# c0gent/hbbft

Hardware: AMD Instinct MI355X
Metric: verified BLS sig shares/sec (whole node) + combine latency, N=64 f=21 (higher is better)
Workload: dtype u32 limbs (Fp, 14x28-bit); 1 GPU; ThresholdSign share verification, BASELINE configs[1]; batch_per_gpu=65536, streams=2, documents_per_gpu=1024, n_nodes=64, f=21, pairing_impl=auto, parallelism=shard-by-batch x1

## Files before the change

### hbbft_amd/csrc/k_pair.hip

```cpp
#define HS_MULFN static __device__ __noinline__
#include "launch.hpp"
#include "pair_side.hpp"

namespace hbs {

template <bool PLUS1>
HP_D H12 h_exp_abs_x(const H12& base) {
  const uint64_t e = PLUS1 ? hb::X_ABS + 1 : hb::X_ABS;
  H12 r = base;
#pragma unroll 1
  for (int k = 62; k >= 0; k--) {
    r = h12_cyclo_sqr(r);
    if ((e >> k) & 1) r = h12_mul(r, base);
  }
  return r;
}
HP_D H12 h_exp_x(const H12& f) { return h12_conj(h_exp_abs_x<false>(f)); }
HP_D H12 h_exp_xm1(const H12& f) { return h12_conj(h_exp_abs_x<true>(f)); }

HP_D H12 h_final_exp(const H12& f, uint32_t* __restrict__ stash) {
  const H12 f1 = h12_mul(h12_conj(f), h12_inv(f));
  const H12 g = h12_mul(h12_frob2(f1), f1);
  stash12(stash, g);
  H12 a = h_exp_xm1(h_exp_xm1(g));
  const H12 b = h12_mul(h_exp_x(a), h12_frob1(a));
  {
    const H12 gs = unstash12(stash);
    const H12 w = h12_mul(h12_mul(h12_frob2(b), h12_conj(b)), h12_mul(h12_cyclo_sqr(gs), gs));
    stash12(stash, w);
  }
  const H12 c = h_exp_x(h_exp_x(b));
  return h12_mul(c, unstash12(stash));
}

template <bool W1, bool W2, int GEN>
__global__ void __launch_bounds__(256, 2) k_pair_verify(PairArgs a) {
  extern __shared__ uint32_t stash_lds[];
  const int i = (int)((blockIdx.x * 256u + threadIdx.x) >> 1);
  if (i >= a.n) return;
  constexpr bool G1 = GEN == 1, G2 = GEN == 2;
  const bool neg2 = (a.flags & 1) != 0;
  SideStateH A, B;
  const bool ok1 = side_init<W1, G1>(a.s1, i, false, A);
  const bool ok2 = side_init<W2, G2>(a.s2, i, neg2, B);
  if (!ok1 || !ok2) {
    if (lp_even() && a.verdict) a.verdict[i] = 0;
    return;
  }
  H12 f = h12_one();
  int step = 0;
#pragma unroll 1
  for (int b = 62; b >= 0; b--) {
    if (b != 62) f = h12_sqr(f);
    {
      const HLine la = side_line<W1, G1, true>(a.s1, A, step, false);
      const HLine lb = side_line<W2, G2, true>(a.s2, B, step, neg2);
      f = h12_mul_lines(f, la.c0, la.c1, la.c4, lb.c0, lb.c1, lb.c4);
    }
    step++;
    if ((hb::X_ABS >> b) & 1) {
      const HLine la = side_line<W1, G1, false>(a.s1, A, step, false);
      const HLine lb = side_line<W2, G2, false>(a.s2, B, step, neg2);
      f = h12_mul_lines(f, la.c0, la.c1, la.c4, lb.c0, lb.c1, lb.c4);
      step++;
    }
  }
  if (a.flags & 2) f = h12_conj(f);
  const H12 e = h_final_exp(f, stash_lds + threadIdx.x);
  if (a.value_out) {
    uint32_t* o = a.value_out + (size_t)i * 144 + (lp_even() ? 0 : 12);
    fp_to_words(e.c0.c0, o + 0);
    fp_to_words(e.c0.c1, o + 24);
    fp_to_words(e.c0.c2, o + 48);
    fp_to_words(e.c1.c0, o + 72);
    fp_to_words(e.c1.c1, o + 96);
    fp_to_words(e.c1.c2, o + 120);
  }
  const bool one = h12_is_one(e);
  if (lp_even() && a.verdict) a.verdict[i] = one ? 1 : 0;
}

}

namespace hbl {

size_t pair_table_bytes(size_t nq) { return nq * (size_t)hbs::PAIR_STEPS * 2 * hbs::PL_Q4 * 16; }

hipError_t pair_verify(hipStream_t s, int n, const PairSideDesc& d1, const PairSideDesc& d2, int flags,
                       uint8_t* verdict, uint32_t* value_out) {
  if (n <= 0) return hipSuccess;
  hbs::PairArgs a;
  a.n = n;
  const PairSideDesc* d[2] = {&d1, &d2};
  hbs::PairSide* o[2] = {&a.s1, &a.s2};
  for (int k = 0; k < 2; k++) {
    o[k]->p = (const uint32_t*)d[k]->p;
    o[k]->q = (const uint32_t*)d[k]->q;
    o[k]->lines = (const int4*)d[k]->lines;
    o[k]->qinf = d[k]->qinf;
    o[k]->idx = d[k]->idx;
    o[k]->nq = (uint32_t)d[k]->nq;
  }
  a.flags = flags;
  a.verdict = verdict;
  a.value_out = value_out;
  const dim3 grid((unsigned)((2 * (size_t)n + 255) / 256)), block(256);
  const size_t lds = (size_t)hbs::STASH_WORDS * 256 * 4;
  const bool w1 = d1.lines == nullptr, w2 = d2.lines == nullptr;
  const int gen = (d1.p == nullptr) == (d2.p == nullptr) ? 0 : (d1.p == nullptr ? 1 : 2);
#define HBS_PAIR_LAUNCH(G)                                                                 \
  do {                                                                                     \
    if (w1 && w2)                                                                          \
      hipLaunchKernelGGL((hbs::k_pair_verify<true, true, G>), grid, block, lds, s, a);     \
    else if (w1)                                                                           \
      hipLaunchKernelGGL((hbs::k_pair_verify<true, false, G>), grid, block, lds, s, a);    \
    else if (w2)                                                                           \
      hipLaunchKernelGGL((hbs::k_pair_verify<false, true, G>), grid, block, lds, s, a);    \
    else                                                                                   \
      hipLaunchKernelGGL((hbs::k_pair_verify<false, false, G>), grid, block, lds, s, a);   \
  } while (0)
  if (gen == 1)
    HBS_PAIR_LAUNCH(1);
  else if (gen == 2)
    HBS_PAIR_LAUNCH(2);
  else
    HBS_PAIR_LAUNCH(0);
#undef HBS_PAIR_LAUNCH
  return hipGetLastError();
}

}
```

### hbbft_amd/csrc/pfp.hpp

```cpp
#pragma once
#include "sfp.hpp"
#include "words.hpp"

#define HP_D __device__ __forceinline__

namespace hbs {

constexpr int DPP_SWAP = 0xB1;
constexpr int DPP_EVEN = 0xA0;
constexpr int DPP_ODD = 0xF5;

HP_D bool lp_even() { return (threadIdx.x & 1) == 0; }
template <int CTRL>
HP_D int32_t dpp(int32_t v) {
  return __builtin_amdgcn_mov_dpp(v, CTRL, 0xF, 0xF, true);
}
template <int CTRL>
HP_D Fp dpp_fp(const Fp& a) {
  Fp r;
#pragma unroll
  for (int i = 0; i < NL; i++) r.l[i] = dpp<CTRL>(a.l[i]);
  return r;
}

HS_MULFN Fp h_mul_l(HS_P14(x), HS_P14(y)) {
  const Fp a = {{HS_L14(x)}};
  const Fp b = {{HS_L14(y)}};
  const int32_t sm = lp_even() ? -1 : 0;
  int32_t Y[NL], W[NL], Z[NL];
#pragma unroll
  for (int i = 0; i < NL; i++) {
    Y[i] = dpp<DPP_EVEN>(b.l[i]);
    W[i] = dpp<DPP_ODD>(b.l[i]);
    Z[i] = (dpp<DPP_SWAP>(a.l[i]) ^ sm) - sm;
  }
  int32_t m[NL];
  int64_t acc = 0;
  Fp r;
#pragma unroll
  for (int k = 0; k < NL; k++) {
#pragma unroll
    for (int i = 0; i <= k; i++) {
      acc += (int64_t)a.l[i] * Y[k - i];
      acc += (int64_t)Z[i] * W[k - i];
    }
#pragma unroll
    for (int i = 0; i < k; i++) acc += (int64_t)m[i] * (int32_t)P_L[k - i];
    m[k] = mont_digit(acc);
    acc += (int64_t)m[k] * (int32_t)P_L[0];
    acc >>= 28;
  }
#pragma unroll
  for (int k = NL; k < 2 * NL - 1; k++) {
#pragma unroll
    for (int i = k - NL + 1; i < NL; i++) {
      acc += (int64_t)a.l[i] * Y[k - i];
      acc += (int64_t)Z[i] * W[k - i];
      acc += (int64_t)m[i] * (int32_t)P_L[k - i];
    }
    r.l[k - NL] = (int32_t)acc & MASK28;
    acc >>= 28;
  }
  r.l[NL - 1] = (int32_t)acc;
  return r;
}

HP_D Fp h_mul(const Fp& a, const Fp& b) { return h_mul_l(HS_E14(a), HS_E14(b)); }

HP_D Fp h_sqr(const Fp& a) {
  const bool ev = lp_even();
  const Fp pa = dpp_fp<DPP_SWAP>(a);
  Fp x, y;
#pragma unroll
  for (int i = 0; i < NL; i++) {
    x.l[i] = pa.l[i] + (ev ? a.l[i] : pa.l[i]);
    y.l[i] = a.l[i] - (ev ? pa.l[i] : 0);
  }
  return fp_mul(x, y);
}

HP_D Fp h_mul_xi(const Fp& a) {
  const int32_t sm = lp_even() ? -1 : 0;
  const Fp pa = dpp_fp<DPP_SWAP>(a);
  Fp r;
#pragma unroll
  for (int i = 0; i < NL; i++) r.l[i] = a.l[i] + ((pa.l[i] ^ sm) - sm);
  fp_norm(r);
  return r;
}
HP_D Fp h_conj(const Fp& a) {
  const Fp n = fp_neg(a);
  return lp_even() ? a : n;
}
HP_D Fp h_zero() { return fp_zero(); }
HP_D Fp h_one() { return lp_even() ? fp_one() : fp_zero(); }
HP_D Fp h_const(const uint32_t (&c0)[NL], const uint32_t (&c1)[NL]) {
  Fp r;
  const bool ev = lp_even();
#pragma unroll
  for (int i = 0; i < NL; i++) r.l[i] = (int32_t)(ev ? c0[i] : c1[i]);
  return r;
}
HP_D bool lp_both(bool v) { return (v ? 1 : 0) & dpp<DPP_SWAP>(v ? 1 : 0); }
HP_D bool h_is_zero(const Fp& a) { return lp_both(fp_is_zero(a)); }
template <int MODE = 0>
HP_D Fp h_inv_vartime(const Fp& a) {
  const Fp s = fp_sqr(a);
  const Fp n = fp_add(s, dpp_fp<DPP_SWAP>(s));
  uint32_t w[12], p[12], r[12];
  fp_to_words(n, w);
  uint32_t nz = 0;
#pragma unroll
  for (int i = 0; i < 12; i++) nz |= w[i];
  if (nz == 0) return fp_zero();
#pragma unroll
  for (int i = 0; i < 12; i++) p[i] = hb::PM2_W[i];
  p[0] += 2;
  hb::words_inv_vartime<12, MODE>(w, p, r);
  return h_conj(fp_mul(a, fp_from_words(r)));
}

template <int M, int K>
HP_D Fp fp_red_mk(const Fp& t, const Fp& a) {
  const int64_t top = (int64_t)t.l[NL - 1] * M + (int64_t)K * a.l[NL - 1];
  const int32_t q = (int32_t)((top * QINV) >> 32);
  Fp r;
  int64_t acc = 0;
#pragma unroll
  for (int i = 0; i < NL - 1; i++) {
    acc += (int64_t)t.l[i] * M + (int64_t)K * a.l[i] - (int64_t)q * (int32_t)P_L[i];
    r.l[i] = (int32_t)acc & MASK28;
    acc >>= 28;
  }
  r.l[NL - 1] = (int32_t)(acc + top - (int64_t)q * (int32_t)P_L[NL - 1]);
  return r;
}
HP_D Fp fp_red_l(const Fp& t) { return fp_red_mk<1, 0>(t, t); }
HP_D Fp h_add_xi_l(const Fp& s, const Fp& t) {
  const int32_t sm = lp_even() ? -1 : 0;
  const Fp pt = dpp_fp<DPP_SWAP>(t);
  Fp r;
#pragma unroll
  for (int i = 0; i < NL; i++) r.l[i] = s.l[i] + t.l[i] + ((pt.l[i] ^ sm) - sm);
  return r;
}
HP_D Fp fp_sub2l(const Fp& a, const Fp& b, const Fp& c) {
  Fp r;
#pragma unroll
  for (int i = 0; i < NL; i++) r.l[i] = a.l[i] - b.l[i] - c.l[i];
  return r;
}

HP_D Fp h_xi_l(const Fp& t) {
  const int32_t sm = lp_even() ? -1 : 0;
  const Fp pt = dpp_fp<DPP_SWAP>(t);
  Fp r;
#pragma unroll
  for (int i = 0; i < NL; i++) r.l[i] = t.l[i] + ((pt.l[i] ^ sm) - sm);
  return r;
}

struct H6 { Fp c0, c1, c2; };
struct H12 { H6 c0, c1; };

HP_D H6 h6_zero() { return {h_zero(), h_zero(), h_zero()}; }
HP_D H6 h6_one() { return {h_one(), h_zero(), h_zero()}; }
HP_D H6 h6_add(const H6& a, const H6& b) { return {fp_add(a.c0, b.c0), fp_add(a.c1, b.c1), fp_add(a.c2, b.c2)}; }
HP_D H6 h6_sub(const H6& a, const H6& b) { return {fp_sub(a.c0, b.c0), fp_sub(a.c1, b.c1), fp_sub(a.c2, b.c2)}; }
HP_D H6 h6_neg(const H6& a) { return {fp_neg(a.c0), fp_neg(a.c1), fp_neg(a.c2)}; }
HP_D H6 h6_red(const H6& a) { return {fp_reduce(a.c0), fp_reduce(a.c1), fp_reduce(a.c2)}; }
HP_D H6 h6_mul_v(const H6& a) { return {h_mul_xi(a.c2), a.c0, a.c1}; }

HP_D H6 h6_mul(const H6& a, const H6& b) {
  const Fp v1 = h_mul(a.c1, b.c1);
  const Fp v2 = h_mul(a.c2, b.c2);
  const Fp d0 = fp_sub2l(h_mul(fp_addl(a.c1, a.c2), fp_add(b.c1, b.c2)), v1, v2);
  const Fp v0 = h_mul(a.c0, b.c0);
  const Fp c0 = fp_red_l(h_add_xi_l(v0, d0));
  const Fp c1 = fp_red_l(h_add_xi_l(fp_sub2l(h_mul(fp_addl(a.c0, a.c1), fp_add(b.c0, b.c1)), v0, v1), v2));
  const Fp c2 = fp_red_l(fp_addl(fp_sub2l(h_mul(fp_addl(a.c0, a.c2), fp_add(b.c0, b.c2)), v0, v2), v1));
  return {c0, c1, c2};
}
HP_D H6 h6_mul_01(const H6& x, const Fp& a, const Fp& b) {
  const Fp t0 = h_mul(x.c0, a);
  const Fp t1 = h_mul(x.c1, b);
  const Fp u = h_mul(x.c2, b);
  const Fp w = h_mul(x.c2, a);
  const Fp s = h_mul(fp_addl(x.c0, x.c1), fp_add(a, b));
  return {fp_add(t0, h_mul_xi(u)), fp_sub(fp_subl(s, t0), t1), fp_add(t1, w)};
}
HP_D H6 h6_mul_1(const H6& x, const Fp& b) {
  const Fp r0 = h_mul(x.c2, b);
  const Fp r1 = h_mul(x.c0, b);
  const Fp r2 = h_mul(x.c1, b);
  return {h_mul_xi(r0), r1, r2};
}
HP_D H6 h6_inv(const H6& a) {
  const Fp c0 = fp_reduce(fp_sub(h_sqr(a.c0), h_mul_xi(h_mul(a.c1, a.c2))));
  const Fp c1 = fp_reduce(fp_sub(h_mul_xi(h_sqr(a.c2)), h_mul(a.c0, a.c1)));
  const Fp c2 = fp_reduce(fp_sub(h_sqr(a.c1), h_mul(a.c0, a.c2)));
  const Fp t = fp_reduce(fp_add(h_mul(a.c0, c0), h_mul_xi(fp_add(h_mul(a.c2, c1), h_mul(a.c1, c2)))));
  const Fp ti = fp_reduce(h_inv_vartime(t));
  return {h_mul(c0, ti), h_mul(c1, ti), h_mul(c2, ti)};
}

HP_D H12 h12_one() { return {h6_one(), h6_zero()}; }
HP_D H12 h12_conj(const H12& a) { return {a.c0, h6_neg(a.c1)}; }
HP_D H12 h12_red(const H12& a) { return {h6_red(a.c0), h6_red(a.c1)}; }
HP_D H12 h12_kcomb(const H6& t0, const H6& t1, const H6& s) {
  return {{fp_red_l(h_add_xi_l(t0.c0, t1.c2)), fp_red_l(fp_addl(t0.c1, t1.c0)), fp_red_l(fp_addl(t0.c2, t1.c1))},
          {fp_red_l(fp_sub2l(s.c0, t0.c0, t1.c0)), fp_red_l(fp_sub2l(s.c1, t0.c1, t1.c1)),
           fp_red_l(fp_sub2l(s.c2, t0.c2, t1.c2))}};
}

HP_D H12 h12_mul(const H12& a, const H12& b) {
  const H6 t0 = h6_mul(a.c0, b.c0);
  const H6 t1 = h6_mul(a.c1, b.c1);
  const H6 s = h6_mul(h6_add(a.c0, a.c1), h6_add(b.c0, b.c1));
  return h12_kcomb(t0, t1, s);
}
HP_D H12 h12_sqr(const H12& a) {
  const H6 t = h6_mul(a.c0, a.c1);
  const H6 s = h6_mul(h6_add(a.c0, a.c1), h6_red(h6_add(a.c0, h6_mul_v(a.c1))));
  return {{fp_red_l(h_add_xi_l(fp_subl(s.c0, t.c0), fp_subl(fp_zero(), t.c2))), fp_red_l(fp_sub2l(s.c1, t.c1, t.c0)),
           fp_red_l(fp_sub2l(s.c2, t.c2, t.c1))},
          {fp_red_l(fp_addl(t.c0, t.c0)), fp_red_l(fp_addl(t.c1, t.c1)), fp_red_l(fp_addl(t.c2, t.c2))}};
}
HP_D H12 h12_mul_014(const H12& f, const Fp& c0, const Fp& c1, const Fp& c4) {
  const H6 fs = h6_add(f.c0, f.c1);
  const Fp c14 = fp_add(c1, c4);
  const H6 t0 = h6_red(h6_mul_01(f.c0, c0, c1));
  const H6 t1 = h6_red(h6_mul_1(f.c1, c4));
  const H6 s = h6_red(h6_mul_01(fs, c0, c14));
  return h12_red({h6_add(t0, h6_mul_v(t1)), h6_sub(h6_sub(s, t0), t1)});
}
HP_D H6 h6_mul_12(const H6& x, const Fp& b1, const Fp& b2) {
  const Fp u = h_mul(x.c1, b1);
  const Fp w = h_mul(x.c2, b2);
  const Fp c0 = fp_red_l(h_xi_l(fp_sub2l(h_mul(fp_addl(x.c1, x.c2), fp_add(b1, b2)), u, w)));
  const Fp c1 = fp_red_l(h_add_xi_l(h_mul(x.c0, b1), w));
  const Fp c2 = fp_red_l(fp_addl(h_mul(x.c0, b2), u));
  return {c0, c1, c2};
}
HP_D H12 h12_mul_lines(const H12& f, const Fp& a0, const Fp& a1, const Fp& a4, const Fp& b0, const Fp& b1,
                       const Fp& b4) {
  const Fp a0b0 = h_mul(a0, b0);
  const Fp a1b1 = h_mul(a1, b1);
  const Fp a4b4 = h_mul(a4, b4);
  const Fp c11 = fp_red_l(fp_sub2l(h_mul(fp_addl(a0, a4), fp_add(b0, b4)), a0b0, a4b4));
  const Fp c12 = fp_red_l(fp_sub2l(h_mul(fp_addl(a1, a4), fp_add(b1, b4)), a1b1, a4b4));
  const H6 C0 = {fp_red_l(h_add_xi_l(a0b0, a4b4)),
                 fp_red_l(fp_sub2l(h_mul(fp_addl(a0, a1), fp_add(b0, b1)), a0b0, a1b1)), a1b1};
  const H6 t0 = h6_mul(f.c0, C0);
  const H6 t1 = h6_mul_12(f.c1, c11, c12);
  const H6 s = h6_mul(h6_add(f.c0, f.c1), {C0.c0, fp_add(C0.c1, c11), fp_add(C0.c2, c12)});
  return h12_kcomb(t0, t1, s);
}
HP_D H12 h12_inv(const H12& a) {
  const H6 t = h6_red(h6_sub(h6_red(h6_mul(a.c0, a.c0)), h6_red(h6_mul_v(h6_red(h6_mul(a.c1, a.c1))))));
  const H6 ti = h6_red(h6_inv(t));
  return h12_red({h6_mul(a.c0, ti), h6_neg(h6_mul(a.c1, ti))});
}

#define HP_FROB1(K) h_const(hb::FROB1_##K##_C0, hb::FROB1_##K##_C1)
HP_D H12 h12_frob1(const H12& f) {
  H12 r;
  r.c0.c0 = h_conj(f.c0.c0);
  r.c1.c0 = h_mul(h_conj(f.c1.c0), HP_FROB1(1));
  r.c0.c1 = h_mul(h_conj(f.c0.c1), HP_FROB1(2));
  r.c1.c1 = h_mul(h_conj(f.c1.c1), HP_FROB1(3));
  r.c0.c2 = h_mul(h_conj(f.c0.c2), HP_FROB1(4));
  r.c1.c2 = h_mul(h_conj(f.c1.c2), HP_FROB1(5));
  return h12_red(r);
}
HP_D H12 h12_frob2(const H12& f) {
  H12 r;
  r.c0.c0 = f.c0.c0;
  r.c1.c0 = fp_mul(f.c1.c0, fp_const(hb::FROB2_1_C0));
  r.c0.c1 = fp_mul(f.c0.c1, fp_const(hb::FROB2_2_C0));
  r.c1.c1 = fp_mul(f.c1.c1, fp_const(hb::FROB2_3_C0));
  r.c0.c2 = fp_mul(f.c0.c2, fp_const(hb::FROB2_4_C0));
  r.c1.c2 = fp_mul(f.c1.c2, fp_const(hb::FROB2_5_C0));
  return r;
}

HP_D H12 h12_cyclo_sqr(const H12& f) {
  const Fp& a0 = f.c0.c0; const Fp& a2 = f.c0.c1; const Fp& a4 = f.c0.c2;
  const Fp& a1 = f.c1.c0; const Fp& a3 = f.c1.c1; const Fp& a5 = f.c1.c2;
  H12 r;
  {
    const Fp s0 = h_sqr(a0), s3 = h_sqr(a3), s03 = h_sqr(fp_add(a0, a3));
    r.c0.c0 = fp_red_mk<3, -2>(h_add_xi_l(s0, s3), a0);
    r.c1.c1 = fp_red_mk<3, 2>(fp_sub2l(s03, s0, s3), a3);
  }
  {
    const Fp s1 = h_sqr(a1), s4 = h_sqr(a4), s14 = h_sqr(fp_add(a1, a4));
    r.c0.c1 = fp_red_mk<3, -2>(h_add_xi_l(s1, s4), a2);
    r.c1.c2 = fp_red_mk<3, 2>(fp_sub2l(s14, s1, s4), a5);
  }
  {
    const Fp s2 = h_sqr(a2), s5 = h_sqr(a5), s25 = h_sqr(fp_add(a2, a5));
    r.c0.c2 = fp_red_mk<3, -2>(h_add_xi_l(s2, s5), a4);
    r.c1.c0 = fp_red_mk<3, 2>(h_add_xi_l(fp_zero(), fp_sub2l(s25, s2, s5)), a1);
  }
  return r;
}

HP_D bool h12_is_one(const H12& f) {
  bool ok = fp_is_zero(fp_sub(f.c0.c0, h_one()));
  ok = ok && fp_is_zero(f.c0.c1) && fp_is_zero(f.c0.c2);
  ok = ok && fp_is_zero(f.c1.c0) && fp_is_zero(f.c1.c1) && fp_is_zero(f.c1.c2);
  return lp_both(ok);
}

struct HJac { Fp x, y, z; };
struct HLine { Fp c0, c1, c4; };

HP_D HLine h_dbl_step(HJac& T) {
  const Fp A = h_sqr(T.x);
  const Fp B = h_sqr(T.y);
  const Fp C = h_sqr(B);
  const Fp D = fp_lin(2, fp_sub(fp_sub(h_sqr(fp_add(T.x, B)), A), C), 0, C);
  const Fp E = fp_lin(3, A, 0, A);
  const Fp ZZ = h_sqr(T.z);
  HLine l;
  l.c0 = fp_sub(h_mul(E, T.x), fp_add(B, B));
  l.c1 = fp_neg(h_mul(E, ZZ));
  const Fp Z3 = fp_sub(fp_sub(h_sqr(fp_add(T.y, T.z)), B), ZZ);
  l.c4 = h_mul(Z3, ZZ);
  const Fp F = h_sqr(E);
  const Fp X3 = fp_sub(F, fp_add(D, D));
  T.y = fp_sub(h_mul(E, fp_sub(D, X3)), fp_lin(8, C, 0, C));
  T.x = X3;
  T.z = Z3;
  l.c0 = fp_reduce(l.c0);
  T.x = fp_reduce(T.x);
  T.y = fp_reduce(T.y);
  T.z = fp_reduce(T.z);
  return l;
}

HP_D HLine h_add_step(HJac& T, const Fp& xQ, const Fp& yQ) {
  const Fp Z1Z1 = h_sqr(T.z);
  const Fp U2 = h_mul(xQ, Z1Z1);
  const Fp S2 = h_mul(h_mul(yQ, T.z), Z1Z1);
  const Fp H = fp_sub(U2, T.x);
  const Fp r = fp_sub(S2, T.y);
  const Fp HH = h_sqr(H);
  const Fp HHH = h_mul(H, HH);
  const Fp V = h_mul(T.x, HH);
  const Fp X3 = fp_sub(fp_sub(h_sqr(r), HHH), fp_add(V, V));
  const Fp Y3 = fp_sub(h_mul(r, fp_sub(V, X3)), h_mul(T.y, HHH));
  const Fp Z3 = h_mul(T.z, H);
  HLine l;
  l.c0 = fp_reduce(fp_sub(h_mul(r, xQ), h_mul(yQ, Z3)));
  l.c1 = fp_neg(r);
  l.c4 = Z3;
  T.x = fp_reduce(X3);
  T.y = fp_reduce(Y3);
  T.z = Z3;
  return l;
}

struct HProj { Fp x, y, z; };

HP_D HLine h_dbl_step_h(HProj& T) {
  const Fp C = h_sqr(T.z);
  const Fp YZ = h_sqr(fp_add(T.y, T.z));
  const Fp B = h_sqr(T.y);
  const Fp H = fp_sub(fp_sub(YZ, B), C);
  const Fp E = fp_red_mk<12, 0>(h_xi_l(C), C);
  const Fp A = h_mul(T.x, T.y);
  const Fp S = h_sqr(T.x);
  HLine l;
  l.c0 = fp_red_mk<1, -1>(B, E);
  l.c1 = fp_lin(-3, S, 0, S);
  l.c4 = H;
  const Fp Bm = fp_lin(1, B, -3, E);
  const Fp Bp = fp_lin(1, B, 3, E);
  T.x = h_mul(fp_addl(A, A), Bm);
  const Fp EE = h_sqr(E);
  T.y = fp_red_mk<1, -12>(h_sqr(Bp), EE);
  const Fp BH = h_mul(fp_addl(B, B), H);
  T.z = fp_red_mk<2, 0>(BH, BH);
  return l;
}

HP_D HLine h_add_step_h(HProj& T, const Fp& xQ, const Fp& yQ) {
  const Fp th = fp_sub(T.y, h_mul(yQ, T.z));
  const Fp la = fp_sub(T.x, h_mul(xQ, T.z));
  HLine l;
  l.c0 = fp_reduce(fp_sub(h_mul(th, xQ), h_mul(la, yQ)));
  l.c1 = fp_neg(th);
  l.c4 = la;
  const Fp C = h_sqr(th);
  const Fp D = h_sqr(la);
  const Fp E = h_mul(la, D);
  const Fp F = h_mul(T.z, C);
  const Fp G = h_mul(T.x, D);
  const Fp H = fp_lin(1, fp_addl(E, F), -2, G);
  const Fp X3 = h_mul(la, H);
  T.y = fp_reduce(fp_sub(h_mul(th, fp_sub(G, H)), h_mul(E, T.y)));
  T.z = h_mul(T.z, E);
  T.x = X3;
  return l;
}

HP_D void h_g2_load(const uint32_t* __restrict__ w, Fp& x, Fp& y) {
  const int o = lp_even() ? 0 : 12;
  x = fp_from_words(w + o);
  y = fp_from_words(w + 24 + o);
}
HP_D bool words_zero(const uint32_t* __restrict__ w, int n) {
  uint32_t o = 0;
  for (int k = 0; k < n; k++) o |= w[k];
  return o == 0;
}

}
```

Before: 3.360 million shares/s.

## Use compressed cyclotomic squaring with batched decompression in final-exp x-powers

Replaces the plain square-and-multiply exponentiation by |x| in the final exponentiation with Karabina-style compressed cyclotomic squaring. Intermediate powers at set bits are parked, then decompressed using a single batched (Montgomery-trick) inversion before being multiplied together. If a denominator is zero, it falls back to the generic routine. This cuts per-squaring field multiplications, at the cost of one inversion per exponentiation, extra parked state that may raise register or scratch pressure, and a noinline call structure.

```diff
diff --git a/hbbft_amd/csrc/k_pair.hip b/hbbft_amd/csrc/k_pair.hip
--- a/hbbft_amd/csrc/k_pair.hip
+++ b/hbbft_amd/csrc/k_pair.hip
@@ -4,32 +4,119 @@
 
 namespace hbs {
 
-template <bool PLUS1>
-HP_D H12 h_exp_abs_x(const H12& base) {
-  const uint64_t e = PLUS1 ? hb::X_ABS + 1 : hb::X_ABS;
-  H12 r = base;
+constexpr int EXP_TOP = 57;
+constexpr uint64_t EXP_HIGH = hb::X_ABS >> EXP_TOP;
+constexpr int EXP_HIGH_BITS = 64 - EXP_TOP;
+constexpr int EXP_NPARK = __builtin_popcountll(hb::X_ABS) - __builtin_popcountll(EXP_HIGH) + 1;
+static_assert((hb::X_ABS & 1) == 0 && (hb::X_ABS >> 63) == 1 && (EXP_HIGH & 1) == 1 && EXP_NPARK >= 1,
+              "the base is no factor of f^|x|, and the power at bit EXP_TOP is the last one parked");
+struct ExpPark {
+  int32_t c[EXP_NPARK][4][NL];
+  int32_t base[6][NL];
+  int32_t pre[EXP_NPARK][NL];
+};
+
+HP_D void park_fp(int32_t (&d)[NL], const Fp& a) {
+#pragma unroll
+  for (int i = 0; i < NL; i++) d[i] = a.l[i];
+}
+HP_D Fp unpark_fp(const int32_t (&s)[NL]) {
+  Fp r;
+#pragma unroll
+  for (int i = 0; i < NL; i++) r.l[i] = s[i];
+  return r;
+}
+HP_D H12 unpark12(const int32_t (&s)[6][NL]) {
+  return {{unpark_fp(s[0]), unpark_fp(s[1]), unpark_fp(s[2])}, {unpark_fp(s[3]), unpark_fp(s[4]), unpark_fp(s[5])}};
+}
+
+static __device__ __noinline__ void h_exp_gs(const ExpPark& pk, bool plus1, H12& out) {
+  const uint64_t e = hb::X_ABS + (plus1 ? 1 : 0);
+  H12 r = unpark12(pk.base);
 #pragma unroll 1
   for (int k = 62; k >= 0; k--) {
     r = h12_cyclo_sqr(r);
-    if ((e >> k) & 1) r = h12_mul(r, base);
+    if ((e >> k) & 1) r = h12_mul(r, unpark12(pk.base));
+  }
+  out = r;
+}
+
+HP_D H12 h_exp_high(const H12& t) {
+  H12 r = t;
+#pragma unroll 1
+  for (int k = EXP_HIGH_BITS - 2; k >= 0; k--) {
+    r = h12_cyclo_sqr(r);
+    if ((EXP_HIGH >> k) & 1) r = h12_mul(r, t);
   }
   return r;
 }
-HP_D H12 h_exp_x(const H12& f) { return h12_conj(h_exp_abs_x<false>(f)); }
-HP_D H12 h_exp_xm1(const H12& f) { return h12_conj(h_exp_abs_x<true>(f)); }
+
+static __device__ __noinline__ bool h_exp_tail(ExpPark& pk, bool plus1, H12& out) {
+  Fp P;
+#pragma unroll 1
+  for (int j = 0; j < EXP_NPARK; j++) {
+    const Fp d = hc_denom(unpark_fp(pk.c[j][0]));
+    if (j == 0) P = d; else P = h_mul(P, d);
+    park_fp(pk.pre[j], P);
+  }
+  if (h_is_zero(P)) return false;
+  Fp I = fp_reduce(h_inv_vartime(P));
+  H12 acc;
+#pragma unroll 1
+  for (int j = EXP_NPARK - 1; j >= (plus1 ? -1 : 0); j--) {
+    H12 E;
+    if (j >= 0) {
+      const HC c = {unpark_fp(pk.c[j][0]), unpark_fp(pk.c[j][1]), unpark_fp(pk.c[j][2]), unpark_fp(pk.c[j][3])};
+      Fp di = I;
+      if (j > 0) {
+        di = h_mul(I, unpark_fp(pk.pre[j - 1]));
+        I = h_mul(I, hc_denom(c.a1));
+      }
+      E = hc_decompress(c, di);
+    } else {
+      E = unpark12(pk.base);
+    }
+    if (j == EXP_NPARK - 1) acc = h_exp_high(E); else acc = h12_mul(acc, E);
+  }
+  out = acc;
+  return true;
+}
+
+template <bool PLUS1>
+HP_D H12 h_exp_abs_x(const H12& base, ExpPark& pk) {
+  park_fp(pk.base[0], base.c0.c0); park_fp(pk.base[1], base.c0.c1); park_fp(pk.base[2], base.c0.c2);
+  park_fp(pk.base[3], base.c1.c0); park_fp(pk.base[4], base.c1.c1); park_fp(pk.base[5], base.c1.c2);
+  HC c = hc_compress(base);
+  int slot = 0;
+#pragma unroll 1
+  for (int k = 1; k <= EXP_TOP; k++) {
+    c = hc_sqr(c);
+    if ((hb::X_ABS >> k) & 1) {
+      park_fp(pk.c[slot][0], c.a1); park_fp(pk.c[slot][1], c.a2);
+      park_fp(pk.c[slot][2], c.a4); park_fp(pk.c[slot][3], c.a5);
+      slot++;
+    }
+  }
+  H12 r;
+  if (!h_exp_tail(pk, PLUS1, r)) h_exp_gs(pk, PLUS1, r);
+  return r;
+}
+HP_D H12 h_exp_x(const H12& f, ExpPark& pk) { return h12_conj(h_exp_abs_x<false>(f, pk)); }
+HP_D H12 h_exp_xm1(const H12& f, ExpPark& pk) { return h12_conj(h_exp_abs_x<true>(f, pk)); }
 
 HP_D H12 h_final_exp(const H12& f, uint32_t* __restrict__ stash) {
   const H12 f1 = h12_mul(h12_conj(f), h12_inv(f));
   const H12 g = h12_mul(h12_frob2(f1), f1);
   stash12(stash, g);
-  H12 a = h_exp_xm1(h_exp_xm1(g));
-  const H12 b = h12_mul(h_exp_x(a), h12_frob1(a));
+  ExpPark pk;
+  H12 a = h_exp_xm1(h_exp_xm1(g, pk), pk);
+  const H12 b = h12_mul(h_exp_x(a, pk), h12_frob1(a));
   {
     const H12 gs = unstash12(stash);
     const H12 w = h12_mul(h12_mul(h12_frob2(b), h12_conj(b)), h12_mul(h12_cyclo_sqr(gs), gs));
     stash12(stash, w);
   }
-  const H12 c = h_exp_x(h_exp_x(b));
+  const H12 c = h_exp_x(h_exp_x(b, pk), pk);
   return h12_mul(c, unstash12(stash));
 }
 
diff --git a/hbbft_amd/csrc/pfp.hpp b/hbbft_amd/csrc/pfp.hpp
--- a/hbbft_amd/csrc/pfp.hpp
+++ b/hbbft_amd/csrc/pfp.hpp
@@ -304,6 +304,35 @@
     r.c1.c0 = fp_red_mk<3, 2>(h_add_xi_l(fp_zero(), fp_sub2l(s25, s2, s5)), a1);
   }
   return r;
+}
+
+struct HC { Fp a1, a2, a4, a5; };
+
+HP_D HC hc_compress(const H12& f) { return {f.c1.c0, f.c0.c1, f.c0.c2, f.c1.c2}; }
+HP_D HC hc_sqr(const HC& c) {
+  HC r;
+  {
+    const Fp s1 = h_sqr(c.a1), s4 = h_sqr(c.a4), s14 = h_sqr(fp_add(c.a1, c.a4));
+    r.a2 = fp_red_mk<3, -2>(h_add_xi_l(s1, s4), c.a2);
+    r.a5 = fp_red_mk<3, 2>(fp_sub2l(s14, s1, s4), c.a5);
+  }
+  {
+    const Fp s2 = h_sqr(c.a2), s5 = h_sqr(c.a5), s25 = h_sqr(fp_add(c.a2, c.a5));
+    r.a4 = fp_red_mk<3, -2>(h_add_xi_l(s2, s5), c.a4);
+    r.a1 = fp_red_mk<3, 2>(h_add_xi_l(fp_zero(), fp_sub2l(s25, s2, s5)), c.a1);
+  }
+  return r;
+}
+HP_D Fp hc_denom(const Fp& a1) { return fp_lin(4, a1, 0, a1); }
+HP_D H12 hc_decompress(const HC& c, const Fp& di) {
+  const Fp s5 = h_sqr(c.a5), s2 = h_sqr(c.a2);
+  Fp t = h_xi_l(s5);
+#pragma unroll
+  for (int i = 0; i < NL; i++) t.l[i] += 3 * s2.l[i];
+  const Fp a3 = h_mul(fp_red_mk<1, -2>(t, c.a4), di);
+  const Fp u = fp_addl(fp_lin(2, h_sqr(a3), -3, h_mul(c.a4, c.a2)), h_mul(c.a1, c.a5));
+  const Fp a0 = fp_red_l(h_add_xi_l(h_one(), u));
+  return {{a0, c.a2, c.a4}, {c.a1, a3, c.a5}};
 }
 
 HP_D bool h12_is_one(const H12& f) {
```

New measurement: 3.493 million shares/s (median of 6 runs). 1.04x the previous value.
